# PaddlePaddle/PaddleRobotics

Measured on AMD Instinct MI355X. Metric: env-steps/sec, 4096 A1 quadrupeds; 1/2/4/8-GPU scaling, higher is better.
Workload: dtype f32

## Files before the change

### paddlerobotics_amd/csrc/etg_core16.h

```cpp
#pragma once

#include <type_traits>

#include "etg_core.h"

namespace etg {

template <class Ctx, class = void> struct sweep_stream_ : std::false_type {};
template <class Ctx> struct sweep_stream_<Ctx, std::void_t<decltype(Ctx::kSweepStream)>> : std::bool_constant<Ctx::kSweepStream> {};
template <class Ctx, class... Args> ETG_HD void run_sweep_stream_(const Ctx& c, Args&&... args) { c.pgs_body_stream(args...); }
template <class Ctx, class = void> struct gram_mfma_ : std::false_type {};
template <class Ctx> struct gram_mfma_<Ctx, std::void_t<decltype(Ctx::kGramMfma)>> : std::bool_constant<Ctx::kGramMfma> {};

template <class F> struct State16 {
  V3<F> p;
  F qx, qy, qz, qw;
  V3<F> wb, vb;
  F q, qd;
  F lam;
  F contact;
  F energy;
  int sweeps;
};

template <class F, class Ctx> ETG_HD State16<F> load_state16(const Ctx& c, const float* base, const float* leg) {
  State16<F> L;
  L.p = {c.ld_env(base, BS_PX), c.ld_env(base, BS_PY), c.ld_env(base, BS_PZ)};
// ... 357 lines not shown
  F mk0[4], mt[4], mk3[4];
#pragma unroll
  for (int lp = 0; lp < 4; lp++) {
    mk0[lp] = ownl[lp] * f0;
    mt[lp] = ownl[lp] * tangf;
    mk3[lp] = ownl[lp] * f3;
  }
  bool anyj = false;
  F jactf = zero, jlo = zero, jhi = zero;
  if (K.jlim) {
    jlo = sel_(s0, F(K.jlo[0]), sel_(s1, F(K.jlo[1]), F(K.jlo[2])));
    jhi = sel_(s0, F(K.jhi[0]), sel_(s1, F(K.jhi[1]), F(K.jhi[2])));
    jactf = mj * sel_((L.q >= jhi) || (L.q <= jlo), one, zero) * live;
    anyj = c.any(jactf > F(0.5f));
  }
  auto finish_tick = [&](auto joints_tag, auto body_tag) {
  constexpr bool joints = decltype(joints_tag)::value;
  constexpr bool body = knee && decltype(body_tag)::value;
  F Ak[4] = {zero, zero, zero, zero};
  if (body) {
#pragma unroll
    for (int lp = 0; lp < 4; lp++) {
      if constexpr (gram) {
        Ak[lp] = Akz[lp];
      } else {
        Ak[lp] = c.rbcast(Z[0], 4 * lp + 3) * Z[0];
#pragma unroll
        for (int k = 1; k < 6; k++) c.fmac_rbcast(Ak[lp], Z[k], Z[k], 4 * lp + 3);
      }
    }
    F ownk = c.qb(hj[0], 3) * Jl0;
    c.fmac_qb(ownk, hj[1], Jl1, 3);
    c.fmac_qb(ownk, hj[2], Jl2, 3);
#pragma unroll
    for (int lp = 0; lp < 4; lp++) Ak[lp] = Ak[lp] + ownl[lp] * ownk;
#pragma unroll
    for (int lp = 0; lp < 4; lp++) c.fmac_rbcast(u, lam, Ak[lp], 4 * lp + 3);
    c.phase_p(10);
  }
  F Z2[6] = {zero, zero, zero, zero, zero, zero}, hj2[3] = {zero, zero, zero};
  constexpr bool b_lds = Ctx::kSlotBLds;
  F sb[32];
#pragma unroll
  for (int k = 0; k < 32; k++) sb[k] = zero;
  F u2s = zero, lam2 = zero, iA2 = zero;
  if constexpr (body) {
    F BA[4][4], BB[4][2], AT[4][2];
    const F rowf2 = tangf * c.qb(rowf, 3);
    V dnb, dir2;
    if (Ctx::kFlat) {
      dnb = Rw.r2;
      dir2 = dir;
// ... 33 lines not shown
#pragma unroll
      for (int lp = 0; lp < 4; lp++)
#pragma unroll
        for (int e = 0; e < 4; e++) BA[lp][e] = Bf[lp][e];
    }
#pragma unroll
    for (int lp = 0; lp < 4; lp++) {
#pragma unroll
      for (int e = 0; e < 4; e++) {
        if constexpr (!gram) {
          BA[lp][e] = c.rbcast(Z[0], 4 * lp + e) * Z2[0];
#pragma unroll
          for (int k = 1; k < 6; k++) c.fmac_rbcast(BA[lp][e], Z[k], Z2[k], 4 * lp + e);
        }
      }
#pragma unroll
      for (int t = 0; t < 2; t++) {
        BB[lp][t] = c.rbcast(Z2[0], 4 * lp + 1 + t) * Z2[0];
        AT[lp][t] = c.rbcast(Z2[0], 4 * lp + 1 + t) * Z[0];
#pragma unroll
        for (int k = 1; k < 6; k++) {
          c.fmac_rbcast(BB[lp][t], Z2[k], Z2[k], 4 * lp + 1 + t);
          c.fmac_rbcast(AT[lp][t], Z2[k], Z[k], 4 * lp + 1 + t);
        }
      }
    }
    F oa[4], ob[2], ot[2];
#pragma unroll
    for (int e = 0; e < 4; e++) oa[e] = c.qb(hj[0], e) * Jb0 + c.qb(hj[1], e) * Jb1 + c.qb(hj[2], e) * Jb2_;
#pragma unroll
    for (int t = 0; t < 2; t++) {
      ob[t] = c.qb(hj2[0], 1 + t) * Jb0 + c.qb(hj2[1], 1 + t) * Jb1 + c.qb(hj2[2], 1 + t) * Jb2_;
      ot[t] = c.qb(hj2[0], 1 + t) * Jl0 + c.qb(hj2[1], 1 + t) * Jl1 + c.qb(hj2[2], 1 + t) * Jl2;
    }
#pragma unroll
    for (int lp = 0; lp < 4; lp++) {
#pragma unroll
      for (int e = 0; e < 4; e++) BA[lp][e] = BA[lp][e] + ownl[lp] * oa[e];
#pragma unroll
      for (int t = 0; t < 2; t++) { BB[lp][t] = BB[lp][t] + ownl[lp] * ob[t]; AT[lp][t] = AT[lp][t] + ownl[lp] * ot[t]; }
    }
    F Add2 = hj2[0] * Jb0 + hj2[1] * Jb1 + hj2[2] * Jb2_;
    Add2 = Add2 + dot(Z2v, Z2v);
    iA2 = sel_(rowf2 > F(0.5f), rcp_(Add2), zero);
#pragma unroll
    for (int lp = 0; lp < 4; lp++) {
#pragma unroll
      for (int e = 0; e < 4; e++) { if (b_lds) c.slotb_st(4 * lp + e, BA[lp][e]); else sb[4 * lp + e] = BA[lp][e]; }
#pragma unroll
      for (int t = 0; t < 2; t++) {
        if (b_lds) { c.slotb_st(16 + 2 * lp + t, BB[lp][t]); c.slotb_st(24 + 2 * lp + t, AT[lp][t]); }
        else { sb[16 + 2 * lp + t] = BB[lp][t]; sb[24 + 2 * lp + t] = AT[lp][t]; }
      }
    }
    c.phase_p(12);
  }
  F sgn = zero, lamq = zero, iAq = zero, c0q = zero;
  F zj[6] = {zero, zero, zero, zero, zero, zero};
  if (joints) {
    F z6[6] = {P.a.x, P.a.y, P.a.z, P.l.x, P.l.y, P.l.z};
    fwd6(s, z6);
    const W zv = cmul(W{{z6[0], z6[1], z6[2]}, {z6[3], z6[4], z6[5]}}, sqv);
#pragma unroll
// ... 8 lines not shown
    constexpr bool pyramid = decltype(pyramid_tag)::value;
    F iAqe = iAq, c0qe = c0q;
    F Bn[8], Bt[8], BBr[4][2], ATr[4][2], u2 = zero;
#pragma unroll
    for (int k = 0; k < 8; k++) Bn[k] = Bt[k] = zero;
#pragma unroll
    for (int lp = 0; lp < 4; lp++) BBr[lp][0] = BBr[lp][1] = ATr[lp][0] = ATr[lp][1] = zero;
    if constexpr (body) {
      F BA[16];
#pragma unroll
      for (int k = 0; k < 16; k++) BA[k] = b_lds ? c.slotb_ld(k) : sb[k];
#pragma unroll
      for (int lp = 0; lp < 4; lp++) {
        Bn[lp] = BA[4 * lp]; Bn[4 + lp] = BA[4 * lp + 3];
        Bt[2 * lp] = BA[4 * lp + 1]; Bt[2 * lp + 1] = BA[4 * lp + 2];
#pragma unroll
        for (int t = 0; t < 2; t++) {
          BBr[lp][t] = b_lds ? c.slotb_ld(16 + 2 * lp + t) : sb[16 + 2 * lp + t];
          ATr[lp][t] = b_lds ? c.slotb_ld(24 + 2 * lp + t) : sb[24 + 2 * lp + t];
        }
      }
      u2 = c.row2_velocity(u2s, lam, BA, lam2, &BBr[0][0]);
    }
    unsigned jrows = 0u;
    if (joints) {
#pragma unroll
      for (int lp = 0; lp < 4; lp++)
#pragma unroll
        for (int e = 0; e < 3; e++) {
          const F me = ownl[lp] * (e == 0 ? f0 : (e == 1 ? f1 : f2));
// ... 48 lines not shown
#pragma unroll
        for (int k = 0; k < 6; k++) du2 = du2 + Z2[k] * (zl[k] - zl0[k]);
        u2 = u2 + du2;
      }
    };
    auto body_friction = [&](F lbn) {
      c.phase_p(8);
      const auto grip2 = lbn > zero;
      const auto gm = c.body_mask(grip2);
      if (!c.mask_any(gm)) return;
      const F lim2 = F(K.body_mu) * lbn;
      if constexpr (Ctx::kAsmSweep && !pyramid) {
        const F iA2g = sel_(grip2, iA2, zero), lim2g = sel_(grip2, lim2, F(1e30f));
#pragma unroll
        for (int lp = 0; lp < 4; lp++) {
          if (!c.mask_leg(gm, lp)) continue;
          c.pgs_pair_body(lam2, u2, u, iA2g, lim2g, ATr[lp][0], ATr[lp][1], BBr[lp][0], BBr[lp][1], mt[lp], lp);
        }
        c.phase_p(11);
        return;
      }
#pragma unroll
      for (int lp = 0; lp < 4; lp++) {
        if (!c.mask_leg(gm, lp)) continue;
        const F lc = lam2 - u2 * iA2;
        F dl;
        if (pyramid) {
          dl = fminf_(fmaxf_(lc, -lim2), lim2) - lam2;
        } else {
          const F sq1 = lc * lc + F(1e-30f);
          const F sc = fminf_(one, lim2 * rsqrt_(sq1 + c.qswap12(sq1)));
          dl = lc * sc - lam2;
        }
        dl = sel_(grip2, dl, zero);
        const F b1 = c.rbcast(dl, 4 * lp + 1), b2 = c.rbcast(dl, 4 * lp + 2);
        u = u + ATr[lp][0] * b1 + ATr[lp][1] * b2;
        u2 = u2 + BBr[lp][0] * b1 + BBr[lp][1] * b2;
        lam2 = lam2 + mt[lp] * dl;
      }
// ... 15 lines not shown
          c.pgs_tangents_disc(lam, u, sel_(grip, iAe, zero), sel_(grip, mue * lnq, F(1e30f)), A, mt);
        }
        return;
      }
#pragma unroll
      for (int lp = 0; lp < 4; lp++) {
        F dln = fmaxf_(-lam, c0e - u * iAe);
        lam = lam + mk0[lp] * dln;
        const F b = c.rbcast(dln, 4 * lp);
        u = u + A[lp][0] * b;
        if (body) u2 = u2 + Bn[lp] * b;
      }
      if (body) {
#pragma unroll
        for (int lp = 0; lp < 4; lp++) {
          F dlk = fmaxf_(-lam, c0e - u * iAe);
          lam = lam + mk3[lp] * dlk;
          F bk = c.rbcast(dlk, 4 * lp + 3);
          u = u + Ak[lp] * bk;
          u2 = u2 + Bn[4 + lp] * bk;
        }
      }
      const F lnq = c.qb(lam, 0);
      const F lim = mue * lnq;
      const auto grip = lnq > zero;
#pragma unroll
      for (int lp = 0; lp < 4; lp++) {
        const F lc = lam - u * iAe;
        F dl;
        if (pyramid) {
// ... 5 lines not shown
        }
        dl = sel_(grip, dl, zero);
        const F b1 = c.rbcast(dl, 4 * lp + 1), b2 = c.rbcast(dl, 4 * lp + 2);
        u = u + A[lp][1] * b1 + A[lp][2] * b2;
        if (body) u2 = u2 + Bt[2 * lp] * b1 + Bt[2 * lp + 1] * b2;
        lam = lam + mt[lp] * dl;
      }
      if constexpr (body) body_friction(c.qb(lam, 3));
    };
    if constexpr (sweep_stream_<Ctx>::value && body && !joints && !pyramid) {
      if (K.res_thr > 0.0f) {
        F tol = F(K.res_sqrt) * iA, tol2 = F(K.res_sqrt) * iA2;
        c.opaque(tol); c.opaque(tol2);
        const unsigned cap = (unsigned)(K.iters > 1 ? K.iters : 1) - 1u;
        unsigned rem = cap;
        run_sweep_stream_(c, lam, u, u2, lam2, rem, iAe, c0e, mue, A, Ak, mk0, mk3, mt, Bn, Bt, iA2, K.body_mu, ATr, BBr, tol, tol2);
        L.sweeps += (int)(cap - rem) + (rem != ~0u ? 1 : 0);
        return;
      }
    }
    if (K.res_thr > 0.0f) {
      F tol = F(K.res_sqrt) * iA, tol2 = F(K.res_sqrt) * iA2;
      if (body) { c.opaque(tol); c.opaque(tol2); }
      const F tolq = F(K.res_sqrt) * iAq;
      int it = 0;
      bool more;
      auto frozen = lam < lam;
      auto sweep_and_test = [&]() {
#ifdef ETG_EAGER_FREEZE
        constexpr bool lazy = false;
#else
// ... 91 lines not shown
  c.opaque3(dl);
  if (body) { dl[0] = dl[0] + hj2[0] * lam2; dl[1] = dl[1] + hj2[1] * lam2; dl[2] = dl[2] + hj2[2] * lam2; }
  const F dj0 = c.qsum(dl[0]), dj1 = c.qsum(dl[1]), dj2 = c.qsum(dl[2]);
  L.qd = mj * (qds + (f0 * dj0 + f1 * dj1 + f2 * dj2) - dot(P, dB));
  if (joints) L.qd = L.qd + mj * (h0 * c.qb(slq, 0) + h1 * c.qb(slq, 1) + h2 * c.qb(slq, 2));
  L.lam = lam;
  const F ln_leg = c.qb(lam, 0);
  L.contact = sel_(act && (ln_leg > zero), one, zero);
#ifdef ETG_TRACE_TICKS
  {
    const F tv[10] = {rowf, phi, lam, lam2, jactf, lamq, bw1 + F(2.0f) * bw2, F((float)L.sweeps), L.q, L.qd};
    c.trace_tick(K, tv);
  }
#endif
  };
  if (anyb) {
    if (anyj) finish_tick(std::true_type{}, std::true_type{});
    else finish_tick(std::false_type{}, std::true_type{});
  } else {
    if (anyj) finish_tick(std::true_type{}, std::false_type{});
    else finish_tick(std::false_type{}, std::false_type{});
  }
  c.phase(9);
  L.q = L.q + dt * L.qd;
  L.p.x = L.p.x + dt * dot(Rw.r0, L.vb);
  L.p.y = L.p.y + dt * dot(Rw.r1, L.vb);
  L.p.z = L.p.z + dt * dot(Rw.r2, L.vb);
  V th = dt * L.wb;
  F a2_ = dot(th, th);
  F sh2 = F(0.5f) - a2_ * (F(1.0f / 48.0f) - a2_ * F(1.0f / 3840.0f));
  F ch2 = one - a2_ * (F(0.125f) - a2_ * (F(1.0f / 384.0f) - a2_ * F(1.0f / 46080.0f)));
  F dx = th.x * sh2, dy = th.y * sh2, dz = th.z * sh2, dw = ch2;
  F nx = L.qw * dx + L.qx * dw + L.qy * dz - L.qz * dy;
  F ny = L.qw * dy - L.qx * dz + L.qy * dw + L.qz * dx;
  F nz = L.qw * dz + L.qx * dy - L.qy * dx + L.qz * dw;
  F nw_ = L.qw * dw - L.qx * dx - L.qy * dy - L.qz * dz;
// ... 458 lines not shown
```

### paddlerobotics_amd/csrc/etg_kernels.hip

```cpp
#include <hip/hip_runtime.h>

#include <string>
#include <vector>

#include "etg_core16.h"
#include "gram16.h"
#include "policy_core.h"
#include "../../include/etgsim_step_policy.h"
#include "../../include/etgsim_collect.h"
#include "../../include/etgsim_monitor.h"
#include "../../include/etgsim_terminal.h"

#ifndef ETG_TU_PARTS
#define ETG_TU_PARTS 1
#define ETG_TU_PART 0
#endif
#define ETG_TU_HOST (ETG_TU_PART == 0)

namespace etg {

template <int CTRL> __device__ __forceinline__ float dpp_(float x) {
  return __int_as_float(__builtin_amdgcn_update_dpp(0, __float_as_int(x), CTRL, 0xF, 0xF, true));
}

// ... 721 lines not shown
        "v_mul_f32_e32 %[sc], %[lim], %[sq]\n"                                                          \
        "v_min_f32_e32 %[sc], 1.0, %[sc]\n"                                                             \
        "v_fma_f32 %[dl], %[lc], %[sc], -%[lam]\n"                                                      \
        "v_fmac_f32_e32 %[lam], %[mk], %[dl]\n"                                                         \
        "s_nop 0\n"                                                                                     \
        "v_fmac_f32_dpp %[u], %[dl], %[at0] row_newbcast:" #R1 ETG_DPPC                                 \
        "v_fmac_f32_dpp %[u2], %[dl], %[bb0] row_newbcast:" #R1 ETG_DPPC                                \
        "v_fmac_f32_dpp %[u], %[dl], %[at1] row_newbcast:" #R2 ETG_DPPC                                 \
        "v_fmac_f32_dpp %[u2], %[dl], %[bb1] row_newbcast:" #R2 ETG_DPPC                                \
        : [lam] "+&v"(lam2), [u2] "+&v"(u2), [u] "+&v"(u), [lc] "=&v"(lc), [sq] "=&v"(sq), [sc] "=&v"(sc), [dl] "=&v"(dl)           \
        : [iA] "v"(iA), [lim] "v"(lim), [at0] "v"(at0), [at1] "v"(at1), [bb0] "v"(bb0), [bb1] "v"(bb1), [mk] "v"(mk))
    switch (lp) { case 0: ETG_PAIRB(1, 2); break; case 1: ETG_PAIRB(5, 6); break; case 2: ETG_PAIRB(9, 10); break; default: ETG_PAIRB(13, 14); break; }
#undef ETG_PAIRB
  }
#if !defined(ETG_SWEEP_BOOKKEEPING_OUTSIDE) && !defined(ETG_NO_ASM_SWEEP) && !defined(ETG_EAGER_FREEZE)
  __device__ __forceinline__ void pgs_body_stream(float& lam, float& u, float& u2, float& lam2, unsigned& rem, float iA, float c0, float mue,
                                                  const float (&A)[4][3], const float* Ak, const float* mk0, const float* mk3, const float* mt,
                                                  const float* bn, const float* bt, float iA2, float body_mu, const float (&AT)[4][2],
                                                  const float (&BB)[4][2], float tol, float tol2) const {
    const unsigned row16 = 0xFFFFu << (tid & 16);
    const unsigned fl = (tid & 32) ? 0u : row16, fh = (tid & 32) ? row16 : 0u;
    float w, wu, wu2, w2, t, dA, dB, lnq, lbn, iAg, limg, lim, lc, sq, sc, iA2g, lim2g, rr;
    unsigned x, gm, tmp;
    unsigned long long live, mv, sa;
#ifdef ETG_FORCE_BODY
#define ETG_SGM "s_or_b32 %[gm], -1, -1\n"
#else
#define ETG_SGM "s_or_b32 %[gm], vcc_lo, vcc_hi\n"
#endif
#define ETG_SU2(D, LP, BOP) "v_fmac_f32_dpp %[wu2], %[" D "], %[" BOP "] row_newbcast:" #LP ETG_DPPC
#define ETG_SROW(D, LP, AOP, MOP, FILL)                                              \
    "v_fma_f32 %[t], -%[wu], %[iA], %[c0]\n"                                         \
    "v_max_f32_e64 %[" D "], -%[w], %[t]\n"                                          \
    "v_fmac_f32_e32 %[w], %[" MOP "], %[" D "]\n"                                    \
    FILL                                                                             \
    "v_fmac_f32_dpp %[wu], %[" D "], %[" AOP "] row_newbcast:" #LP ETG_DPPC
#define ETG_SPAIR(D, R1, R2, A1, A2, MOP, F1, F2, F3)                                \
    "v_fma_f32 %[lc], -%[wu], %[iAg], %[w]\n"                                        \
    "v_fmaak_f32 %[sq], %[lc], %[lc], 0x0da24260\n"                                  \
// ... 15 lines not shown
    "v_fmaak_f32 %[sq], %[lc], %[lc], 0x0da24260\n"                                  \
    "s_nop 1\n"                                                                      \
    "v_add_f32_dpp %[sq], %[sq], %[sq] quad_perm:[0,2,1,3]" ETG_DPPC                 \
    "v_rsq_f32_e32 %[sq], %[sq]\n"                                                   \
    "s_nop 0\n"                                                                      \
    "v_mul_f32_e32 %[sc], %[lim2g], %[sq]\n"                                         \
    "v_min_f32_e32 %[sc], 1.0, %[sc]\n"                                              \
    "v_fma_f32 %[dA], %[lc], %[sc], -%[w2]\n"                                        \
    "v_fmac_f32_e32 %[w2], %[" MOP "], %[dA]\n"                                      \
    "s_nop 0\n"                                                                      \
    "v_fmac_f32_dpp %[wu], %[dA], %[at" #LP "0] row_newbcast:" #R1 ETG_DPPC          \
    "v_fmac_f32_dpp %[wu2], %[dA], %[bb" #LP "0] row_newbcast:" #R1 ETG_DPPC         \
    "v_fmac_f32_dpp %[wu], %[dA], %[at" #LP "1] row_newbcast:" #R2 ETG_DPPC          \
    "v_fmac_f32_dpp %[wu2], %[dA], %[bb" #LP "1] row_newbcast:" #R2 ETG_DPPC         \
    ".Letg_sw_leg" #LP "_%=:\n"
    asm volatile(
        "s_mov_b64 vcc, -1\n"
        ".Letg_sw_top_%=:\n"
        "v_mov_b32_e32 %[wu2], %[u2]\n"
        "v_fma_f32 %[t], -%[u], %[iA], %[c0]\n"
        "v_max_f32_e64 %[dA], -%[lam], %[t]\n"
        "v_fma_f32 %[w], %[m0], %[dA], %[lam]\n"
        "v_mov_b32_e32 %[wu], %[u]\n"
        "v_fmac_f32_dpp %[wu], %[dA], %[a0] row_newbcast:0" ETG_DPPC
        ETG_SROW("dB", 4, "a1", "m1", ETG_SU2("dA", 0, "b0"))
        ETG_SROW("dA", 8, "a2", "m2", ETG_SU2("dB", 4, "b1"))
        ETG_SROW("dB", 12, "a3", "m3", ETG_SU2("dA", 8, "b2"))
        ETG_SROW("dA", 3, "k0", "n0", ETG_SU2("dB", 12, "b3"))
        ETG_SROW("dB", 7, "k1", "n1", ETG_SU2("dA", 3, "b4"))
        ETG_SROW("dA", 11, "k2", "n2", ETG_SU2("dB", 7, "b5"))
        ETG_SROW("dB", 15, "k3", "n3", ETG_SU2("dA", 11, "b6"))
        ETG_SU2("dB", 15, "b7")
        "v_mov_b32_dpp %[lnq], %[w] quad_perm:[0,0,0,0]" ETG_DPPC
        "v_mov_b32_dpp %[lbn], %[w] quad_perm:[3,3,3,3]" ETG_DPPC
        "v_cmp_lt_f32_e64 %[sa], 0, %[lnq]\n"
        "v_mul_f32_e32 %[lim], %[mue], %[lnq]\n"
        "v_cndmask_b32_e64 %[iAg], 0, %[iA], %[sa]\n"
        "v_cndmask_b32_e64 %[limg], %[big], %[lim], %[sa]\n"
        ETG_SPAIR("dA", 1, 2, "a01", "a02", "t0",
                  "v_and_b32_e32 %[x], vcc_lo, %[fl]\n" "v_and_or_b32 %[x], vcc_hi, %[fh], %[x]\n",
                  "v_cmp_ne_u32_e64 %[live], 0, %[x]\n",
                  "v_mov_b32_e32 %[w2], %[lam2]\n")
        ETG_SPAIR("dB", 5, 6, "a11", "a12", "t1", ETG_SU2("dA", 1, "e0") ETG_SU2("dA", 2, "e1"),
                  "v_cmp_lt_f32_e32 vcc, 0, %[lbn]\n",
                  "v_mul_f32_e32 %[lim], %[bmu], %[lbn]\n")
        ETG_SPAIR("dA", 9, 10, "a21", "a22", "t2", ETG_SU2("dB", 5, "e2") ETG_SU2("dB", 6, "e3"),
                  "v_cndmask_b32_e32 %[iA2g], 0, %[iA2], vcc\n",
                  "v_cndmask_b32_e32 %[lim2g], %[big], %[lim], vcc\n")
        ETG_SPAIR("dB", 13, 14, "a31", "a32", "t3", ETG_SU2("dA", 9, "e4") ETG_SU2("dA", 10, "e5"),
                  ETG_SGM,
                  "v_sub_f32_e32 %[rr], %[w], %[lam]\n")
        ETG_SU2("dB", 13, "e6") ETG_SU2("dB", 14, "e7")
        "v_cmp_gt_f32_e64 %[mv], |%[rr]|, %[tol]\n"
        "s_cbranch_scc0 .Letg_sw_nf_%=\n"
        ETG_SLEG(0, "0x000f000f", 1, 2, "t0")
        ETG_SLEG(1, "0x00f000f0", 5, 6, "t1")
        ETG_SLEG(2, "0x0f000f00", 9, 10, "t2")
        ETG_SLEG(3, "0xf000f000", 13, 14, "t3")
        "v_sub_f32_e32 %[rr], %[w2], %[lam2]\n"
        "v_cmp_gt_f32_e64 %[sa], |%[rr]|, %[tol2]\n"
        "s_or_b64 %[mv], %[mv], %[sa]\n"
        "v_cndmask_b32_e64 %[lam2], %[lam2], %[w2], %[live]\n"
        ".Letg_sw_nf_%=:\n"
        "v_cndmask_b32_e64 %[lam], %[lam], %[w], %[live]\n"
        "v_cndmask_b32_e64 %[u], %[u], %[wu], %[live]\n"
        "v_cndmask_b32_e64 %[u2], %[u2], %[wu2], %[live]\n"
        "s_and_b64 vcc, %[mv], %[live]\n"
        "s_cbranch_scc0 .Letg_sw_end_%=\n"
        "s_sub_u32 %[rem], %[rem], 1\n"
        "s_cbranch_scc0 .Letg_sw_top_%=\n"
        ".Letg_sw_end_%=:\n"
        : [lam] "+&v"(lam), [u] "+&v"(u), [u2] "+&v"(u2), [lam2] "+&v"(lam2), [rem] "+&s"(rem), [w] "=&v"(w), [wu] "=&v"(wu), [wu2] "=&v"(wu2),
          [w2] "=&v"(w2), [t] "=&v"(t), [dA] "=&v"(dA), [dB] "=&v"(dB), [lnq] "=&v"(lnq), [lbn] "=&v"(lbn), [iAg] "=&v"(iAg), [limg] "=&v"(limg),
          [lim] "=&v"(lim), [lc] "=&v"(lc), [sq] "=&v"(sq), [sc] "=&v"(sc), [iA2g] "=&v"(iA2g), [lim2g] "=&v"(lim2g), [rr] "=&v"(rr), [x] "=&v"(x),
          [gm] "=&s"(gm), [tmp] "=&s"(tmp), [live] "=&s"(live), [mv] "=&s"(mv), [sa] "=&s"(sa)
        : [iA] "v"(iA), [c0] "v"(c0), [mue] "v"(mue), [big] "v"(1e30f), [a0] "v"(A[0][0]), [a1] "v"(A[1][0]), [a2] "v"(A[2][0]), [a3] "v"(A[3][0]),
          [m0] "v"(mk0[0]), [m1] "v"(mk0[1]), [m2] "v"(mk0[2]), [m3] "v"(mk0[3]),
          [k0] "v"(Ak[0]), [k1] "v"(Ak[1]), [k2] "v"(Ak[2]), [k3] "v"(Ak[3]),
          [n0] "v"(mk3[0]), [n1] "v"(mk3[1]), [n2] "v"(mk3[2]), [n3] "v"(mk3[3]),
          [b0] "v"(bn[0]), [b1] "v"(bn[1]), [b2] "v"(bn[2]), [b3] "v"(bn[3]), [b4] "v"(bn[4]), [b5] "v"(bn[5]), [b6] "v"(bn[6]), [b7] "v"(bn[7]),
          [a01] "v"(A[0][1]), [a02] "v"(A[0][2]), [a11] "v"(A[1][1]), [a12] "v"(A[1][2]), [a21] "v"(A[2][1]), [a22] "v"(A[2][2]),
          [a31] "v"(A[3][1]), [a32] "v"(A[3][2]), [t0] "v"(mt[0]), [t1] "v"(mt[1]), [t2] "v"(mt[2]), [t3] "v"(mt[3]),
          [e0] "v"(bt[0]), [e1] "v"(bt[1]), [e2] "v"(bt[2]), [e3] "v"(bt[3]), [e4] "v"(bt[4]), [e5] "v"(bt[5]), [e6] "v"(bt[6]), [e7] "v"(bt[7]),
          [iA2] "v"(iA2), [bmu] "s"(body_mu), [at00] "v"(AT[0][0]), [at01] "v"(AT[0][1]), [at10] "v"(AT[1][0]), [at11] "v"(AT[1][1]),
          [at20] "v"(AT[2][0]), [at21] "v"(AT[2][1]), [at30] "v"(AT[3][0]), [at31] "v"(AT[3][1]),
          [bb00] "v"(BB[0][0]), [bb01] "v"(BB[0][1]), [bb10] "v"(BB[1][0]), [bb11] "v"(BB[1][1]),
          [bb20] "v"(BB[2][0]), [bb21] "v"(BB[2][1]), [bb30] "v"(BB[3][0]), [bb31] "v"(BB[3][1]),
          [tol] "v"(tol), [tol2] "v"(tol2), [fl] "v"(fl), [fh] "v"(fh)
        : "vcc", "scc");
#undef ETG_SGM
#undef ETG_SU2
#undef ETG_SROW
#undef ETG_SPAIR
#undef ETG_SLEG
  }
#endif
#undef ETG_DPPC
  __device__ __forceinline__ void dpp_ready10(float* z, float* hj, float* lam) const {
    asm volatile("s_nop 1" : "+v"(z[0]), "+v"(z[1]), "+v"(z[2]), "+v"(z[3]), "+v"(z[4]), "+v"(z[5]), "+v"(hj[0]), "+v"(hj[1]), "+v"(hj[2]), "+v"(lam[0]));
  }
  __device__ __forceinline__ static int slotb_field(int k) { return k < 30 ? PR_LINK + k : PR_KP + (k - 30); }
  __device__ __forceinline__ void slotb_st(int k, float v) const { const_cast<float*>(lds)[slotb_field(k) * 64] = v; }
  __device__ __forceinline__ float slotb_ld(int k) const { return lds[slotb_field(k) * 64]; }
  __device__ __forceinline__ void opaque(float& v) const { asm volatile("" : "+v"(v)); }
  __device__ __forceinline__ void opaque3(float* v) const { asm volatile("" : "+v"(v[0]), "+v"(v[1]), "+v"(v[2])); }
  __device__ __forceinline__ void dpp_ready(float* v, int n) const {
    if (n == 6) asm volatile("s_nop 1" : "+v"(v[0]), "+v"(v[1]), "+v"(v[2]), "+v"(v[3]), "+v"(v[4]), "+v"(v[5]));
    else if (n == 3) asm volatile("s_nop 1" : "+v"(v[0]), "+v"(v[1]), "+v"(v[2]));
    else asm volatile("s_nop 1" : "+v"(v[0]));
  }
// ... 55 lines not shown
  static constexpr bool kStepLocal = false;
#ifdef ETG_NO_ASM_SWEEP
  static constexpr bool kAsmSweep = false;
#else
  static constexpr bool kAsmSweep = true;
#endif
#ifdef ETG_GRAM_DPP
  static constexpr bool kGramMfma = false;
#else
  static constexpr bool kGramMfma = true;
#endif
#if defined(ETG_NO_ASM_SWEEP) || defined(ETG_SWEEP_BOOKKEEPING_OUTSIDE) || defined(ETG_EAGER_FREEZE)
  static constexpr bool kSweepStream = false;
#else
  static constexpr bool kSweepStream = true;
#endif
};

template <bool FLAT, bool KNEE, bool PLAIN> struct GpuCtx16W : GpuCtx16T<FLAT, KNEE, PLAIN> {
  static constexpr bool kStepLocal = true;
  __device__ __forceinline__ float tpar(int k) const { return this->lds[k * 64]; }
  __device__ __forceinline__ float tpar_joint(int base) const { return this->lds[(base + this->sc) * 64]; }
  __device__ __forceinline__ float tpar_link(int k) const { return this->sub < 3 ? this->lds[(PR_LINK + 10 * this->sub + k) * 64] : 0.0f; }
};
constexpr int PARK16 = 36;
__device__ __forceinline__ void park16(float* p, const State16<float>& L, const StepCtl16<float>& S) {
  const float v[PARK16] = {L.p.x, L.p.y, L.p.z, L.qx, L.qy, L.qz, L.qw, L.wb.x, L.wb.y, L.wb.z, L.vb.x, L.vb.y, L.vb.z, L.q, L.qd, L.lam, L.contact,
                           __int_as_float(S.step_count), __int_as_float(S.tick), __int_as_float(S.has_last), S.last, S.lbx, S.lby, S.lbz, S.last_fwx,
                           S.ret, S.len, S.r0, S.r1, S.r2, S.fx0, S.fx1, S.fy0, S.fy1, 0.0f, 0.0f};
#pragma unroll
// ... 2080 lines not shown
```

Before: 48.31 million.

## Specialize body-contact solve tail when only one leg's knee touches

Adds a compile-time leg index to the finish_tick path. When exactly one leg has an active knee/body contact row and no joint limits are active, a specialized variant runs instead of the general one. That variant skips the Gram, BB/AT, store/load and PGS pair updates for the other three legs, and uses a trimmed inline-asm sweep loop that handles only that leg's row. The aim is to cut per-iteration ALU, DPP and LDS work in the common single-knee-contact case. The cost is four extra template instantiations, which means more code size and instruction-cache pressure, plus a wave-uniform mask check to pick the variant.

New measurement: 48.37 million (median of 5 runs). Within noise of the previous version (+0.1%).

```diff
diff --git a/paddlerobotics_amd/csrc/etg_core16.h b/paddlerobotics_amd/csrc/etg_core16.h
--- a/paddlerobotics_amd/csrc/etg_core16.h
+++ b/paddlerobotics_amd/csrc/etg_core16.h
@@ -11,6 +11,13 @@
 template <class Ctx, class... Args> ETG_HD void run_sweep_stream_(const Ctx& c, Args&&... args) { c.pgs_body_stream(args...); }
 template <class Ctx, class = void> struct gram_mfma_ : std::false_type {};
 template <class Ctx> struct gram_mfma_<Ctx, std::void_t<decltype(Ctx::kGramMfma)>> : std::bool_constant<Ctx::kGramMfma> {};
+template <class Ctx, class = void> struct one_leg_tail_ : std::false_type {};
+#ifdef ETG_ONE_LEG_TAIL_ALL
+template <class Ctx> struct one_leg_tail_<Ctx, std::void_t<decltype(&Ctx::body_mask), decltype(&Ctx::mask_leg)>> : std::true_type {};
+#else
+template <class Ctx> struct one_leg_tail_<Ctx, std::void_t<decltype(Ctx::kOneLegTail)>> : std::bool_constant<Ctx::kOneLegTail> {};
+#endif
+template <int B, class Ctx, class... Args> ETG_HD void run_sweep_stream1_(const Ctx& c, Args&&... args) { c.template pgs_body_stream1<B>(args...); }
 
 template <class F> struct State16 {
   V3<F> p;
@@ -398,13 +405,17 @@
     jactf = mj * sel_((L.q >= jhi) || (L.q <= jlo), one, zero) * live;
     anyj = c.any(jactf > F(0.5f));
   }
-  auto finish_tick = [&](auto joints_tag, auto body_tag) {
+  auto finish_tick = [&](auto joints_tag, auto body_tag, auto leg_tag) {
   constexpr bool joints = decltype(joints_tag)::value;
   constexpr bool body = knee && decltype(body_tag)::value;
+  constexpr int leg = decltype(leg_tag)::value;
+  static_assert(leg < 0 || decltype(body_tag)::value, "a one-leg tail is a body tail");
+  auto leg_on = [](int lp) { return leg < 0 || lp == leg; };
   F Ak[4] = {zero, zero, zero, zero};
   if (body) {
 #pragma unroll
     for (int lp = 0; lp < 4; lp++) {
+      if (!leg_on(lp)) continue;
       if constexpr (gram) {
         Ak[lp] = Akz[lp];
       } else {
@@ -417,9 +428,9 @@
     c.fmac_qb(ownk, hj[1], Jl1, 3);
     c.fmac_qb(ownk, hj[2], Jl2, 3);
 #pragma unroll
-    for (int lp = 0; lp < 4; lp++) Ak[lp] = Ak[lp] + ownl[lp] * ownk;
-#pragma unroll
-    for (int lp = 0; lp < 4; lp++) c.fmac_rbcast(u, lam, Ak[lp], 4 * lp + 3);
+    for (int lp = 0; lp < 4; lp++) if (leg_on(lp)) Ak[lp] = Ak[lp] + ownl[lp] * ownk;
+#pragma unroll
+    for (int lp = 0; lp < 4; lp++) if (leg_on(lp)) c.fmac_rbcast(u, lam, Ak[lp], 4 * lp + 3);
     c.phase_p(10);
   }
   F Z2[6] = {zero, zero, zero, zero, zero, zero}, hj2[3] = {zero, zero, zero};
@@ -483,6 +494,7 @@
           for (int k = 1; k < 6; k++) c.fmac_rbcast(BA[lp][e], Z[k], Z2[k], 4 * lp + e);
         }
       }
+      if (!leg_on(lp)) continue;
 #pragma unroll
       for (int t = 0; t < 2; t++) {
         BB[lp][t] = c.rbcast(Z2[0], 4 * lp + 1 + t) * Z2[0];
@@ -506,6 +518,7 @@
     for (int lp = 0; lp < 4; lp++) {
 #pragma unroll
       for (int e = 0; e < 4; e++) BA[lp][e] = BA[lp][e] + ownl[lp] * oa[e];
+      if (!leg_on(lp)) continue;
 #pragma unroll
       for (int t = 0; t < 2; t++) { BB[lp][t] = BB[lp][t] + ownl[lp] * ob[t]; AT[lp][t] = AT[lp][t] + ownl[lp] * ot[t]; }
     }
@@ -516,6 +529,7 @@
     for (int lp = 0; lp < 4; lp++) {
 #pragma unroll
       for (int e = 0; e < 4; e++) { if (b_lds) c.slotb_st(4 * lp + e, BA[lp][e]); else sb[4 * lp + e] = BA[lp][e]; }
+      if (!leg_on(lp)) continue;
 #pragma unroll
       for (int t = 0; t < 2; t++) {
         if (b_lds) { c.slotb_st(16 + 2 * lp + t, BB[lp][t]); c.slotb_st(24 + 2 * lp + t, AT[lp][t]); }
@@ -554,6 +568,7 @@
       for (int lp = 0; lp < 4; lp++) {
         Bn[lp] = BA[4 * lp]; Bn[4 + lp] = BA[4 * lp + 3];
         Bt[2 * lp] = BA[4 * lp + 1]; Bt[2 * lp + 1] = BA[4 * lp + 2];
+        if (!leg_on(lp)) continue;
 #pragma unroll
         for (int t = 0; t < 2; t++) {
           BBr[lp][t] = b_lds ? c.slotb_ld(16 + 2 * lp + t) : sb[16 + 2 * lp + t];
@@ -632,7 +647,7 @@
         const F iA2g = sel_(grip2, iA2, zero), lim2g = sel_(grip2, lim2, F(1e30f));
 #pragma unroll
         for (int lp = 0; lp < 4; lp++) {
-          if (!c.mask_leg(gm, lp)) continue;
+          if (!leg_on(lp) || !c.mask_leg(gm, lp)) continue;
           c.pgs_pair_body(lam2, u2, u, iA2g, lim2g, ATr[lp][0], ATr[lp][1], BBr[lp][0], BBr[lp][1], mt[lp], lp);
         }
         c.phase_p(11);
@@ -640,7 +655,7 @@
       }
 #pragma unroll
       for (int lp = 0; lp < 4; lp++) {
-        if (!c.mask_leg(gm, lp)) continue;
+        if (!leg_on(lp) || !c.mask_leg(gm, lp)) continue;
         const F lc = lam2 - u2 * iA2;
         F dl;
         if (pyramid) {
@@ -686,6 +701,7 @@
       if (body) {
 #pragma unroll
         for (int lp = 0; lp < 4; lp++) {
+          if (!leg_on(lp)) continue;
           F dlk = fmaxf_(-lam, c0e - u * iAe);
           lam = lam + mk3[lp] * dlk;
           F bk = c.rbcast(dlk, 4 * lp + 3);
@@ -721,7 +737,10 @@
         c.opaque(tol); c.opaque(tol2);
         const unsigned cap = (unsigned)(K.iters > 1 ? K.iters : 1) - 1u;
         unsigned rem = cap;
-        run_sweep_stream_(c, lam, u, u2, lam2, rem, iAe, c0e, mue, A, Ak, mk0, mk3, mt, Bn, Bt, iA2, K.body_mu, ATr, BBr, tol, tol2);
+        if constexpr (leg >= 0)
+          run_sweep_stream1_<leg>(c, lam, u, u2, lam2, rem, iAe, c0e, mue, A, Ak, mk0, mk3, mt, Bn, Bt, iA2, K.body_mu, ATr, BBr, tol, tol2);
+        else
+          run_sweep_stream_(c, lam, u, u2, lam2, rem, iAe, c0e, mue, A, Ak, mk0, mk3, mt, Bn, Bt, iA2, K.body_mu, ATr, BBr, tol, tol2);
         L.sweeps += (int)(cap - rem) + (rem != ~0u ? 1 : 0);
         return;
       }
@@ -843,12 +862,32 @@
   }
 #endif
   };
+  using any_leg = std::integral_constant<int, -1>;
   if (anyb) {
-    if (anyj) finish_tick(std::true_type{}, std::true_type{});
-    else finish_tick(std::false_type{}, std::true_type{});
+    if (anyj) {
+      finish_tick(std::true_type{}, std::true_type{}, any_leg{});
+    } else {
+      int legb = -1;
+      if constexpr (knee && one_leg_tail_<Ctx>::value) {
+        const auto m = c.body_mask((rowf * f3) > F(0.5f));
+        const bool in0 = c.mask_leg(m, 0), in1 = c.mask_leg(m, 1), in2 = c.mask_leg(m, 2), in3 = c.mask_leg(m, 3);
+        if ((int)in0 + (int)in1 + (int)in2 + (int)in3 == 1) legb = in0 ? 0 : (in1 ? 1 : (in2 ? 2 : 3));
+      }
+      if constexpr (knee && one_leg_tail_<Ctx>::value) {
+        switch (legb) {
+          case 0: finish_tick(std::false_type{}, std::true_type{}, std::integral_constant<int, 0>{}); break;
+          case 1: finish_tick(std::false_type{}, std::true_type{}, std::integral_constant<int, 1>{}); break;
+          case 2: finish_tick(std::false_type{}, std::true_type{}, std::integral_constant<int, 2>{}); break;
+          case 3: finish_tick(std::false_type{}, std::true_type{}, std::integral_constant<int, 3>{}); break;
+          default: finish_tick(std::false_type{}, std::true_type{}, any_leg{}); break;
+        }
+      } else {
+        finish_tick(std::false_type{}, std::true_type{}, any_leg{});
+      }
+    }
   } else {
-    if (anyj) finish_tick(std::true_type{}, std::false_type{});
-    else finish_tick(std::false_type{}, std::false_type{});
+    if (anyj) finish_tick(std::true_type{}, std::false_type{}, any_leg{});
+    else finish_tick(std::false_type{}, std::false_type{}, any_leg{});
   }
   c.phase(9);
   L.q = L.q + dt * L.qd;
diff --git a/paddlerobotics_amd/csrc/etg_kernels.hip b/paddlerobotics_amd/csrc/etg_kernels.hip
--- a/paddlerobotics_amd/csrc/etg_kernels.hip
+++ b/paddlerobotics_amd/csrc/etg_kernels.hip
@@ -759,15 +759,6 @@
 #undef ETG_PAIRB
   }
 #if !defined(ETG_SWEEP_BOOKKEEPING_OUTSIDE) && !defined(ETG_NO_ASM_SWEEP) && !defined(ETG_EAGER_FREEZE)
-  __device__ __forceinline__ void pgs_body_stream(float& lam, float& u, float& u2, float& lam2, unsigned& rem, float iA, float c0, float mue,
-                                                  const float (&A)[4][3], const float* Ak, const float* mk0, const float* mk3, const float* mt,
-                                                  const float* bn, const float* bt, float iA2, float body_mu, const float (&AT)[4][2],
-                                                  const float (&BB)[4][2], float tol, float tol2) const {
-    const unsigned row16 = 0xFFFFu << (tid & 16);
-    const unsigned fl = (tid & 32) ? 0u : row16, fh = (tid & 32) ? row16 : 0u;
-    float w, wu, wu2, w2, t, dA, dB, lnq, lbn, iAg, limg, lim, lc, sq, sc, iA2g, lim2g, rr;
-    unsigned x, gm, tmp;
-    unsigned long long live, mv, sa;
 #ifdef ETG_FORCE_BODY
 #define ETG_SGM "s_or_b32 %[gm], -1, -1\n"
 #else
@@ -813,86 +804,143 @@
     "v_fmac_f32_dpp %[wu], %[dA], %[at" #LP "1] row_newbcast:" #R2 ETG_DPPC          \
     "v_fmac_f32_dpp %[wu2], %[dA], %[bb" #LP "1] row_newbcast:" #R2 ETG_DPPC         \
     ".Letg_sw_leg" #LP "_%=:\n"
+#define ETG_STREAM_HEAD                                                                                                  \
+        "s_mov_b64 vcc, -1\n"                                         \
+        ".Letg_sw_top_%=:\n"                                                                                             \
+                                                  \
+        "v_mov_b32_e32 %[wu2], %[u2]\n"                                                                                  \
+        "v_fma_f32 %[t], -%[u], %[iA], %[c0]\n"                                                                          \
+        "v_max_f32_e64 %[dA], -%[lam], %[t]\n"                                                                           \
+        "v_fma_f32 %[w], %[m0], %[dA], %[lam]\n"                      \
+        "v_mov_b32_e32 %[wu], %[u]\n"                                                                                    \
+        "v_fmac_f32_dpp %[wu], %[dA], %[a0] row_newbcast:0" ETG_DPPC                                                     \
+        ETG_SROW("dB", 4, "a1", "m1", ETG_SU2("dA", 0, "b0"))                                                            \
+        ETG_SROW("dA", 8, "a2", "m2", ETG_SU2("dB", 4, "b1"))                                                            \
+        ETG_SROW("dB", 12, "a3", "m3", ETG_SU2("dA", 8, "b2"))
+#define ETG_STREAM_MID                                                                                                   \
+             \
+        "v_mov_b32_dpp %[lnq], %[w] quad_perm:[0,0,0,0]" ETG_DPPC                                                        \
+        "v_mov_b32_dpp %[lbn], %[w] quad_perm:[3,3,3,3]" ETG_DPPC                                                        \
+        "v_cmp_lt_f32_e64 %[sa], 0, %[lnq]\n"                                                                            \
+        "v_mul_f32_e32 %[lim], %[mue], %[lnq]\n"                                                                         \
+        "v_cndmask_b32_e64 %[iAg], 0, %[iA], %[sa]\n"                                                                    \
+        "v_cndmask_b32_e64 %[limg], %[big], %[lim], %[sa]\n"                                                             \
+         \
+        ETG_SPAIR("dA", 1, 2, "a01", "a02", "t0",                                                                        \
+                  "v_and_b32_e32 %[x], vcc_lo, %[fl]\n" "v_and_or_b32 %[x], vcc_hi, %[fh], %[x]\n",                      \
+                  "v_cmp_ne_u32_e64 %[live], 0, %[x]\n",                                                                 \
+                  "v_mov_b32_e32 %[w2], %[lam2]\n")                                                                      \
+        ETG_SPAIR("dB", 5, 6, "a11", "a12", "t1", ETG_SU2("dA", 1, "e0") ETG_SU2("dA", 2, "e1"),                         \
+                  "v_cmp_lt_f32_e32 vcc, 0, %[lbn]\n",                                                                   \
+                  "v_mul_f32_e32 %[lim], %[bmu], %[lbn]\n")                                                              \
+        ETG_SPAIR("dA", 9, 10, "a21", "a22", "t2", ETG_SU2("dB", 5, "e2") ETG_SU2("dB", 6, "e3"),                        \
+                  "v_cndmask_b32_e32 %[iA2g], 0, %[iA2], vcc\n",                                                         \
+                  "v_cndmask_b32_e32 %[lim2g], %[big], %[lim], vcc\n")                                                   \
+        ETG_SPAIR("dB", 13, 14, "a31", "a32", "t3", ETG_SU2("dA", 9, "e4") ETG_SU2("dA", 10, "e5"),                      \
+                  ETG_SGM,                                                                                               \
+                  "v_sub_f32_e32 %[rr], %[w], %[lam]\n")                                                                 \
+        ETG_SU2("dB", 13, "e6") ETG_SU2("dB", 14, "e7")                                                                  \
+        "v_cmp_gt_f32_e64 %[mv], |%[rr]|, %[tol]\n"                                                                      \
+        "s_cbranch_scc0 .Letg_sw_nf_%=\n"
+#define ETG_STREAM_TAIL                                                                                                  \
+        "v_sub_f32_e32 %[rr], %[w2], %[lam2]\n"                                                                          \
+        "v_cmp_gt_f32_e64 %[sa], |%[rr]|, %[tol2]\n"                                                                     \
+        "s_or_b64 %[mv], %[mv], %[sa]\n"                                                                                 \
+        "v_cndmask_b32_e64 %[lam2], %[lam2], %[w2], %[live]\n"                                                           \
+        ".Letg_sw_nf_%=:\n"                                                                                              \
+            \
+        "v_cndmask_b32_e64 %[lam], %[lam], %[w], %[live]\n"                                                              \
+        "v_cndmask_b32_e64 %[u], %[u], %[wu], %[live]\n"                                                                 \
+        "v_cndmask_b32_e64 %[u2], %[u2], %[wu2], %[live]\n"                                                              \
+        "s_and_b64 vcc, %[mv], %[live]\n"                                                                                \
+        "s_cbranch_scc0 .Letg_sw_end_%=\n"                            \
+        "s_sub_u32 %[rem], %[rem], 1\n"                                                                                  \
+        "s_cbranch_scc0 .Letg_sw_top_%=\n"                            \
+        ".Letg_sw_end_%=:\n"
+#define ETG_STREAM_OUT                                                                                                   \
+          [lam] "+&v"(lam), [u] "+&v"(u), [u2] "+&v"(u2), [lam2] "+&v"(lam2), [rem] "+&s"(rem), [w] "=&v"(w), [wu] "=&v"(wu), [wu2] "=&v"(wu2), \
+          [w2] "=&v"(w2), [t] "=&v"(t), [dA] "=&v"(dA), [dB] "=&v"(dB), [lnq] "=&v"(lnq), [lbn] "=&v"(lbn), [iAg] "=&v"(iAg), [limg] "=&v"(limg), \
+          [lim] "=&v"(lim), [lc] "=&v"(lc), [sq] "=&v"(sq), [sc] "=&v"(sc), [iA2g] "=&v"(iA2g), [lim2g] "=&v"(lim2g), [rr] "=&v"(rr), [x] "=&v"(x), \
+          [gm] "=&s"(gm), [tmp] "=&s"(tmp), [live] "=&s"(live), [mv] "=&s"(mv), [sa] "=&s"(sa)
+#define ETG_STREAM_IN                                                                                                    \
+          [iA] "v"(iA), [c0] "v"(c0), [mue] "v"(mue), [big] "v"(1e30f), [a0] "v"(A[0][0]), [a1] "v"(A[1][0]), [a2] "v"(A[2][0]), [a3] "v"(A[3][0]), \
+          [m0] "v"(mk0[0]), [m1] "v"(mk0[1]), [m2] "v"(mk0[2]), [m3] "v"(mk0[3]),                                        \
+          [b0] "v"(bn[0]), [b1] "v"(bn[1]), [b2] "v"(bn[2]), [b3] "v"(bn[3]),                                            \
+          [a01] "v"(A[0][1]), [a02] "v"(A[0][2]), [a11] "v"(A[1][1]), [a12] "v"(A[1][2]), [a21] "v"(A[2][1]), [a22] "v"(A[2][2]), \
+          [a31] "v"(A[3][1]), [a32] "v"(A[3][2]), [t0] "v"(mt[0]), [t1] "v"(mt[1]), [t2] "v"(mt[2]), [t3] "v"(mt[3]),    \
+          [e0] "v"(bt[0]), [e1] "v"(bt[1]), [e2] "v"(bt[2]), [e3] "v"(bt[3]), [e4] "v"(bt[4]), [e5] "v"(bt[5]), [e6] "v"(bt[6]), [e7] "v"(bt[7]), \
+          [iA2] "v"(iA2), [bmu] "s"(body_mu), [tol] "v"(tol), [tol2] "v"(tol2), [fl] "v"(fl), [fh] "v"(fh)
+#define ETG_STREAM_VARS                                                                                                  \
+    const unsigned row16 = 0xFFFFu << (tid & 16);                                                                        \
+    const unsigned fl = (tid & 32) ? 0u : row16, fh = (tid & 32) ? row16 : 0u;                                           \
+    float w, wu, wu2, w2, t, dA, dB, lnq, lbn, iAg, limg, lim, lc, sq, sc, iA2g, lim2g, rr;                              \
+    unsigned x, gm, tmp;                                                                                                 \
+    unsigned long long live, mv, sa
+  __device__ __forceinline__ void pgs_body_stream(float& lam, float& u, float& u2, float& lam2, unsigned& rem, float iA, float c0, float mue,
+                                                  const float (&A)[4][3], const float* Ak, const float* mk0, const float* mk3, const float* mt,
+                                                  const float* bn, const float* bt, float iA2, float body_mu, const float (&AT)[4][2],
+                                                  const float (&BB)[4][2], float tol, float tol2) const {
+    ETG_STREAM_VARS;
     asm volatile(
-        "s_mov_b64 vcc, -1\n"
-        ".Letg_sw_top_%=:\n"
-        "v_mov_b32_e32 %[wu2], %[u2]\n"
-        "v_fma_f32 %[t], -%[u], %[iA], %[c0]\n"
-        "v_max_f32_e64 %[dA], -%[lam], %[t]\n"
-        "v_fma_f32 %[w], %[m0], %[dA], %[lam]\n"
-        "v_mov_b32_e32 %[wu], %[u]\n"
-        "v_fmac_f32_dpp %[wu], %[dA], %[a0] row_newbcast:0" ETG_DPPC
-        ETG_SROW("dB", 4, "a1", "m1", ETG_SU2("dA", 0, "b0"))
-        ETG_SROW("dA", 8, "a2", "m2", ETG_SU2("dB", 4, "b1"))
-        ETG_SROW("dB", 12, "a3", "m3", ETG_SU2("dA", 8, "b2"))
+        ETG_STREAM_HEAD
         ETG_SROW("dA", 3, "k0", "n0", ETG_SU2("dB", 12, "b3"))
         ETG_SROW("dB", 7, "k1", "n1", ETG_SU2("dA", 3, "b4"))
         ETG_SROW("dA", 11, "k2", "n2", ETG_SU2("dB", 7, "b5"))
         ETG_SROW("dB", 15, "k3", "n3", ETG_SU2("dA", 11, "b6"))
         ETG_SU2("dB", 15, "b7")
-        "v_mov_b32_dpp %[lnq], %[w] quad_perm:[0,0,0,0]" ETG_DPPC
-        "v_mov_b32_dpp %[lbn], %[w] quad_perm:[3,3,3,3]" ETG_DPPC
-        "v_cmp_lt_f32_e64 %[sa], 0, %[lnq]\n"
-        "v_mul_f32_e32 %[lim], %[mue], %[lnq]\n"
-        "v_cndmask_b32_e64 %[iAg], 0, %[iA], %[sa]\n"
-        "v_cndmask_b32_e64 %[limg], %[big], %[lim], %[sa]\n"
-        ETG_SPAIR("dA", 1, 2, "a01", "a02", "t0",
-                  "v_and_b32_e32 %[x], vcc_lo, %[fl]\n" "v_and_or_b32 %[x], vcc_hi, %[fh], %[x]\n",
-                  "v_cmp_ne_u32_e64 %[live], 0, %[x]\n",
-                  "v_mov_b32_e32 %[w2], %[lam2]\n")
-        ETG_SPAIR("dB", 5, 6, "a11", "a12", "t1", ETG_SU2("dA", 1, "e0") ETG_SU2("dA", 2, "e1"),
-                  "v_cmp_lt_f32_e32 vcc, 0, %[lbn]\n",
-                  "v_mul_f32_e32 %[lim], %[bmu], %[lbn]\n")
-        ETG_SPAIR("dA", 9, 10, "a21", "a22", "t2", ETG_SU2("dB", 5, "e2") ETG_SU2("dB", 6, "e3"),
-                  "v_cndmask_b32_e32 %[iA2g], 0, %[iA2], vcc\n",
-                  "v_cndmask_b32_e32 %[lim2g], %[big], %[lim], vcc\n")
-        ETG_SPAIR("dB", 13, 14, "a31", "a32", "t3", ETG_SU2("dA", 9, "e4") ETG_SU2("dA", 10, "e5"),
-                  ETG_SGM,
-                  "v_sub_f32_e32 %[rr], %[w], %[lam]\n")
-        ETG_SU2("dB", 13, "e6") ETG_SU2("dB", 14, "e7")
-        "v_cmp_gt_f32_e64 %[mv], |%[rr]|, %[tol]\n"
-        "s_cbranch_scc0 .Letg_sw_nf_%=\n"
+        ETG_STREAM_MID
         ETG_SLEG(0, "0x000f000f", 1, 2, "t0")
         ETG_SLEG(1, "0x00f000f0", 5, 6, "t1")
         ETG_SLEG(2, "0x0f000f00", 9, 10, "t2")
         ETG_SLEG(3, "0xf000f000", 13, 14, "t3")
-        "v_sub_f32_e32 %[rr], %[w2], %[lam2]\n"
-        "v_cmp_gt_f32_e64 %[sa], |%[rr]|, %[tol2]\n"
-        "s_or_b64 %[mv], %[mv], %[sa]\n"
-        "v_cndmask_b32_e64 %[lam2], %[lam2], %[w2], %[live]\n"
-        ".Letg_sw_nf_%=:\n"
-        "v_cndmask_b32_e64 %[lam], %[lam], %[w], %[live]\n"
-        "v_cndmask_b32_e64 %[u], %[u], %[wu], %[live]\n"
-        "v_cndmask_b32_e64 %[u2], %[u2], %[wu2], %[live]\n"
-        "s_and_b64 vcc, %[mv], %[live]\n"
-        "s_cbranch_scc0 .Letg_sw_end_%=\n"
-        "s_sub_u32 %[rem], %[rem], 1\n"
-        "s_cbranch_scc0 .Letg_sw_top_%=\n"
-        ".Letg_sw_end_%=:\n"
-        : [lam] "+&v"(lam), [u] "+&v"(u), [u2] "+&v"(u2), [lam2] "+&v"(lam2), [rem] "+&s"(rem), [w] "=&v"(w), [wu] "=&v"(wu), [wu2] "=&v"(wu2),
-          [w2] "=&v"(w2), [t] "=&v"(t), [dA] "=&v"(dA), [dB] "=&v"(dB), [lnq] "=&v"(lnq), [lbn] "=&v"(lbn), [iAg] "=&v"(iAg), [limg] "=&v"(limg),
-          [lim] "=&v"(lim), [lc] "=&v"(lc), [sq] "=&v"(sq), [sc] "=&v"(sc), [iA2g] "=&v"(iA2g), [lim2g] "=&v"(lim2g), [rr] "=&v"(rr), [x] "=&v"(x),
-          [gm] "=&s"(gm), [tmp] "=&s"(tmp), [live] "=&s"(live), [mv] "=&s"(mv), [sa] "=&s"(sa)
-        : [iA] "v"(iA), [c0] "v"(c0), [mue] "v"(mue), [big] "v"(1e30f), [a0] "v"(A[0][0]), [a1] "v"(A[1][0]), [a2] "v"(A[2][0]), [a3] "v"(A[3][0]),
-          [m0] "v"(mk0[0]), [m1] "v"(mk0[1]), [m2] "v"(mk0[2]), [m3] "v"(mk0[3]),
+        ETG_STREAM_TAIL
+        : ETG_STREAM_OUT
+        : ETG_STREAM_IN,
           [k0] "v"(Ak[0]), [k1] "v"(Ak[1]), [k2] "v"(Ak[2]), [k3] "v"(Ak[3]),
           [n0] "v"(mk3[0]), [n1] "v"(mk3[1]), [n2] "v"(mk3[2]), [n3] "v"(mk3[3]),
-          [b0] "v"(bn[0]), [b1] "v"(bn[1]), [b2] "v"(bn[2]), [b3] "v"(bn[3]), [b4] "v"(bn[4]), [b5] "v"(bn[5]), [b6] "v"(bn[6]), [b7] "v"(bn[7]),
-          [a01] "v"(A[0][1]), [a02] "v"(A[0][2]), [a11] "v"(A[1][1]), [a12] "v"(A[1][2]), [a21] "v"(A[2][1]), [a22] "v"(A[2][2]),
-          [a31] "v"(A[3][1]), [a32] "v"(A[3][2]), [t0] "v"(mt[0]), [t1] "v"(mt[1]), [t2] "v"(mt[2]), [t3] "v"(mt[3]),
-          [e0] "v"(bt[0]), [e1] "v"(bt[1]), [e2] "v"(bt[2]), [e3] "v"(bt[3]), [e4] "v"(bt[4]), [e5] "v"(bt[5]), [e6] "v"(bt[6]), [e7] "v"(bt[7]),
-          [iA2] "v"(iA2), [bmu] "s"(body_mu), [at00] "v"(AT[0][0]), [at01] "v"(AT[0][1]), [at10] "v"(AT[1][0]), [at11] "v"(AT[1][1]),
+          [b4] "v"(bn[4]), [b5] "v"(bn[5]), [b6] "v"(bn[6]), [b7] "v"(bn[7]),
+          [at00] "v"(AT[0][0]), [at01] "v"(AT[0][1]), [at10] "v"(AT[1][0]), [at11] "v"(AT[1][1]),
           [at20] "v"(AT[2][0]), [at21] "v"(AT[2][1]), [at30] "v"(AT[3][0]), [at31] "v"(AT[3][1]),
           [bb00] "v"(BB[0][0]), [bb01] "v"(BB[0][1]), [bb10] "v"(BB[1][0]), [bb11] "v"(BB[1][1]),
-          [bb20] "v"(BB[2][0]), [bb21] "v"(BB[2][1]), [bb30] "v"(BB[3][0]), [bb31] "v"(BB[3][1]),
-          [tol] "v"(tol), [tol2] "v"(tol2), [fl] "v"(fl), [fh] "v"(fh)
+          [bb20] "v"(BB[2][0]), [bb21] "v"(BB[2][1]), [bb30] "v"(BB[3][0]), [bb31] "v"(BB[3][1])
         : "vcc", "scc");
+  }
+  template <int B>
+  __device__ __forceinline__ void pgs_body_stream1(float& lam, float& u, float& u2, float& lam2, unsigned& rem, float iA, float c0, float mue,
+                                                   const float (&A)[4][3], const float* Ak, const float* mk0, const float* mk3, const float* mt,
+                                                   const float* bn, const float* bt, float iA2, float body_mu, const float (&AT)[4][2],
+                                                   const float (&BB)[4][2], float tol, float tol2) const {
+    static_assert(B >= 0 && B < 4, "leg index");
+    ETG_STREAM_VARS;
+#define ETG_STREAM1(LANE, LEGBITS, R1, R2, MOP)                                                                          \
+    asm volatile(                                                                                                        \
+        ETG_STREAM_HEAD                                                                                                  \
+        ETG_SROW("dA", LANE, "kx", "nx", ETG_SU2("dB", 12, "b3"))                                                        \
+        ETG_SU2("dA", LANE, "bx")                                                                                        \
+        ETG_STREAM_MID                                                                                                   \
+        ETG_SLEG(x, LEGBITS, R1, R2, MOP)                                                                                \
+        ETG_STREAM_TAIL                                                                                                  \
+        : ETG_STREAM_OUT                                                                                                 \
+        : ETG_STREAM_IN, [kx] "v"(Ak[B]), [nx] "v"(mk3[B]), [bx] "v"(bn[4 + B]),                                         \
+          [atx0] "v"(AT[B][0]), [atx1] "v"(AT[B][1]), [bbx0] "v"(BB[B][0]), [bbx1] "v"(BB[B][1])                         \
+        : "vcc", "scc")
+    if constexpr (B == 0) ETG_STREAM1(3, "0x000f000f", 1, 2, "t0");
+    else if constexpr (B == 1) ETG_STREAM1(7, "0x00f000f0", 5, 6, "t1");
+    else if constexpr (B == 2) ETG_STREAM1(11, "0x0f000f00", 9, 10, "t2");
+    else ETG_STREAM1(15, "0xf000f000", 13, 14, "t3");
+#undef ETG_STREAM1
+  }
+#undef ETG_STREAM_HEAD
+#undef ETG_STREAM_MID
+#undef ETG_STREAM_TAIL
+#undef ETG_STREAM_OUT
+#undef ETG_STREAM_IN
+#undef ETG_STREAM_VARS
 #undef ETG_SGM
 #undef ETG_SU2
 #undef ETG_SROW
 #undef ETG_SPAIR
 #undef ETG_SLEG
-  }
 #endif
 #undef ETG_DPPC
   __device__ __forceinline__ void dpp_ready10(float* z, float* hj, float* lam) const {
@@ -978,6 +1026,11 @@
   static constexpr bool kSweepStream = false;
 #else
   static constexpr bool kSweepStream = true;
+#endif
+#ifdef ETG_NO_ONE_LEG_TAIL
+  static constexpr bool kOneLegTail = false;
+#else
+  static constexpr bool kOneLegTail = true;
 #endif
 };
 
```
